# cnkuangshi/LightCTR

Hardware: AMD Instinct MI355X
Metric: examples/sec (whole node), FM training on synthetic Criteo-shaped sparse (higher is better)
Workload: dtype fp32; 1 GPU; model=FM k=16, ftrl fused update, global_batch=65536, num_features=16777216, num_fields=39, parallelism=single-gpu, hipGraph

## Files before the change

lightctr_amd/models/fm.py:

```python

from __future__ import annotations

from dataclasses import dataclass

import torch

from ..ops import fm_ref
from ..ops._extension import require_hip_ops, sort_ids, sort_ids_rec
from ..utils.checks import validate_csr_batch
from ..utils.metrics import auc_score


@dataclass
class FMHyper:
    num_features: int
    k: int = 16
    optimizer: str = "adagrad"
    lr: float = 0.1
    eps: float = 1e-8
    l2: float = 1e-5
    ftrl_alpha: float = 0.15
    ftrl_beta: float = 1.0
    ftrl_l1: float = 1e-4
    ftrl_l2: float = 1e-4
    ftrl_v: str = "adagrad"
    init_sigma: float = 0.01
    seed: int = 1234


class FMModel:

    def __init__(self, hyper: FMHyper, device: str = "cpu",
                 max_batch_nnz: int = 1 << 22):
        self.h = hyper
        self.device = torch.device(device)
        F, K = hyper.num_features, hyper.k
        assert K in (4, 8, 16, 32, 64), "K must divide the 64-lane wavefront"
        g = torch.Generator().manual_seed(hyper.seed)
        self.W = torch.zeros(F, device=self.device)
        self.V = (
            torch.randn(F, K, generator=g) * hyper.init_sigma
        ).to(self.device)
        self.gradW = torch.zeros_like(self.W)
        self.gradV = torch.zeros_like(self.V)
        self.nW = torch.zeros_like(self.W)
        self.nV = torch.zeros_like(self.V)
        if hyper.optimizer == "ftrl":
            self.zW = torch.zeros_like(self.W)
            self.zV = torch.zeros_like(self.V)
        nwords = (F + 63) // 64
        self.touched = torch.zeros(nwords, dtype=torch.int64, device=self.device)
        cap = min(F, max_batch_nnz)
        self.uniq = torch.zeros(cap, dtype=torch.int32, device=self.device)
        self.count = torch.zeros(1, dtype=torch.int32, device=self.device)
        self._use_hip = self.device.type == "cuda"
        self.backward_mode = "segment"
        self.segment_cap = 256
        self.fused_apply = False
        self.sort_impl = "onesweep"
        self.sort_status = torch.zeros(1, dtype=torch.int32,
                                       device=self.device)
        if self._use_hip:
            require_hip_ops()

    def forward(self, row_ptr, fids, vals):
        if self._use_hip:
            ops = require_hip_ops()
            pred, sumVX = ops.fm_forward(row_ptr, fids, vals, self.W, self.V)
        else:
            pred, sumVX = fm_ref.fm_forward_ref(row_ptr, fids, vals, self.W, self.V)
        return pred, sumVX

    def predict_proba(self, row_ptr, fids, vals):
        pred, _ = self.forward(row_ptr, fids, vals)
        return torch.sigmoid(torch.clamp(pred, -16, 16))

    def train_step(self, row_ptr, fids, vals, labels) -> torch.Tensor:
        B = row_ptr.numel() - 1
        scale = 1.0 / B
        validate_csr_batch(row_ptr, fids, vals, self.h.num_features)
        if self._use_hip:
            ops = require_hip_ops()
            if (self.backward_mode in ("segment", "segment_list")
                    and not self.fused_apply):
                tiled = (self.backward_mode == "segment"
                         and self._cap_tiles(ops))
                loss, dpred, sumVX, rec = ops.fm_forward_train(
                    row_ptr, fids, vals, self.W, self.V, labels, scale,
                    reset=self.count if tiled else None)
                self._segment_backward(ops, fids, sumVX, dpred, rec, tiled)
                return loss
            pred, sumVX = ops.fm_forward(row_ptr, fids, vals, self.W, self.V)
            loss, dpred = ops.logloss_grad(pred, labels, scale)
            if (self.backward_mode == "segment_emit"
                    and not self.fused_apply):
                self._segment_emit_backward(ops, row_ptr, fids, vals, sumVX,
                                            dpred)
                return loss
            if self.backward_mode in ("sorted", "segment", "segment_list",
                                      "segment_emit"):
                sorted_fids, perm = sort_ids(fids, self.h.num_features)
                gw, gv = ops.fm_backward_emit(row_ptr, fids, vals, self.V,
                                              sumVX, dpred)
                if self.fused_apply:
                    if (self.h.optimizer == "ftrl"
                            and self.h.ftrl_v == "adagrad"):
                        ops.fm_sorted_apply_fused(
                            sorted_fids, perm, gw, gv, self.gradW,
                            self.gradV, self.touched, self.W, self.V,
                            self.nW, self.nV, self.zW, None, 3,
                            self.h.ftrl_alpha, self.h.ftrl_beta,
                            self.h.ftrl_l1, self.h.ftrl_l2,
                            v_lr=self.h.lr, v_eps=self.h.eps,
                            v_l2=self.h.l2)
                    elif self.h.optimizer == "ftrl":
                        ops.fm_sorted_apply_fused(
                            sorted_fids, perm, gw, gv, self.gradW,
                            self.gradV, self.touched, self.W, self.V,
                            self.nW, self.nV, self.zW, self.zV, 2,
# ... 57 lines not shown
                                 self.h.lr, self.h.eps, self.h.l2)

    def _cap_tiles(self, ops) -> bool:
        tile, cap = ops.fm_segment_tile(), int(self.segment_cap)
        return cap <= tile and tile % cap == 0

    def _segment_pieces(self, ops, sorted_fids, worklist=True):
        nnz = sorted_fids.numel()
        cap = int(self.segment_cap)
        if worklist:
            lists = tuple(ops.segment_worklist(sorted_fids, cap, self.count))
        else:
            lists = (cap,)
        spill = self.uniq[: min(self.uniq.numel(), nnz // cap + 1)]
        mode = self._opt_mode()
        if mode == 1:
            knobs = (self.h.lr, self.h.eps, self.h.l2, 0.0)
        else:
            knobs = (self.h.ftrl_alpha, self.h.ftrl_beta, self.h.ftrl_l1,
                     self.h.ftrl_l2)
        tail = (*lists, self.gradW, self.gradV, spill,
                self.count, self.W, self.V, self.nW, self.nV,
                self.zW if mode != 1 else None,
                self.zV if mode == 2 else None, mode, *knobs)
        kw = dict(v_lr=self.h.lr, v_eps=self.h.eps, v_l2=self.h.l2)
        return spill, tail, kw

    def _segment_backward(self, ops, fids, sumVX, dpred, rec, tiled):
        if fids.numel() == 0:
            return
        sorted_fids, sorted_rec = sort_ids_rec(
            fids, rec, self.h.num_features, impl=self.sort_impl,
            status=self.sort_status)
        spill, tail, kw = self._segment_pieces(ops, sorted_fids,
                                               worklist=not tiled)
        reduce = (ops.fm_segment_tile_rec if tiled
                  else ops.fm_segment_apply_rec)
        reduce(sorted_fids, sorted_rec, sumVX, dpred, *tail, **kw)
        self._sparse_apply(ops, spill)

    def _segment_emit_backward(self, ops, row_ptr, fids, vals, sumVX, dpred):
        if fids.numel() == 0:
            return
        sorted_fids, perm = sort_ids(fids, self.h.num_features)
        gw, gv = ops.fm_backward_emit(row_ptr, fids, vals, self.V, sumVX,
                                      dpred)
        spill, tail, kw = self._segment_pieces(ops, sorted_fids)
        ops.fm_segment_apply(sorted_fids, perm, tail[0], tail[1], gw, gv,
                             *tail[2:], **kw)
        self._sparse_apply(ops, spill)

    def state_dict(self) -> dict:
        d = {"W": self.W, "V": self.V, "nW": self.nW, "nV": self.nV,
             "hyper": self.h.__dict__}
        if self.h.optimizer == "ftrl":
            d["zW"], d["zV"] = self.zW, self.zV
        return d

    def save(self, path: str) -> None:
        torch.save(self.state_dict(), path)

    def load(self, path: str) -> None:
        d = torch.load(path, map_location=self.device, weights_only=True)
        self.W.copy_(d["W"])
        self.V.copy_(d["V"])
        self.nW.copy_(d["nW"])
# ... 44 lines not shown
```

lightctr_amd/ops/_extension.py:

```python

from __future__ import annotations

import torch

_hip_ops = None
_import_error: Exception | None = None

try:
    from . import _hip_ops as _ext

    _hip_ops = _ext
except ImportError as e:
    _import_error = e


def has_hip_ops() -> bool:
    return _hip_ops is not None


def require_hip_ops():
    if _hip_ops is None:
        raise ImportError(
            "lightctr_amd HIP extension (_hip_ops) is not built but a GPU "
            "op was requested. Build it in-tree with "
            "`PYTORCH_ROCM_ARCH=gfx950 python setup.py build_ext --inplace`. "
            f"Original import error: {_import_error!r}"
        )
    return _hip_ops


class _LazyOps:

    def __getattr__(self, name):
        return getattr(require_hip_ops(), name)


hip_ops = _LazyOps()


def sort_ids(fids, upper: int):
    end_bit = max(1, int(upper - 1).bit_length())
    return require_hip_ops().radix_sort_index(fids, end_bit)


def sort_ids_rec(fids, rec, upper: int, impl: str = "onesweep", status=None):
    if impl not in ("onesweep", "rocprim"):
        raise ValueError(f"unknown sort impl {impl!r}")
    ops = require_hip_ops()
    end_bit = max(1, int(upper - 1).bit_length())
    if impl == "onesweep" and end_bit <= 31 and fids.numel() < (1 << 30):
        return ops.onesweep_sort_rec(fids, rec, end_bit, status)
    return ops.radix_sort_rec(fids, rec, end_bit)
```

lightctr_amd/ops/csrc/bindings.cpp:

```cpp
#include <torch/extension.h>
#include <ATen/cuda/CUDAContext.h>
#include <c10/cuda/CUDAException.h>

#include <cstdint>
#include <cstdio>
#include <cstdlib>
#include <cstring>
#include <limits>
#include <stdexcept>
#include <string>
#include <vector>

#include "launchers.h"

namespace {

#define CHK(x, ...) TORCH_CHECK(x, __VA_ARGS__)

void check_cuda_f32(const at::Tensor& t, const char* name) {
  CHK(t.is_cuda(), name, " must be on GPU");
  CHK(t.scalar_type() == at::kFloat, name, " must be fp32");
  CHK(t.is_contiguous(), name, " must be contiguous");
}

void check_cuda_i32(const at::Tensor& t, const char* name) {
  CHK(t.is_cuda(), name, " must be on GPU");
  CHK(t.scalar_type() == at::kInt, name, " must be int32");
  CHK(t.is_contiguous(), name, " must be contiguous");
}

void check_embed_k(int64_t K) {
  CHK(K == 4 || K == 8 || K == 16 || K == 32 || K == 64,
      "latent width K must be one of 4, 8, 16, 32, 64, got ", K);
}
// ... 1165 lines not shown
}

std::vector<at::Tensor> onesweep_sort_rec(at::Tensor keys, at::Tensor rec,
                                          int64_t end_bit,
                                          c10::optional<at::Tensor> status) {
  check_cuda_i32(keys, "keys");
  CHK(end_bit >= 1 && end_bit <= 31, "end_bit in [1,31]");
  CHK(keys.numel() < (1L << 30), "n must be below 2^30");
  const int n = (int)keys.numel();
  check_cuda_rec(rec, n, "rec");
  if (status.has_value()) {
    check_cuda_i32(*status, "status");
    CHK(status->numel() >= 1, "status must hold one word");
  }
  auto sorted = at::empty_like(keys);
  auto sorted_rec = at::empty_like(rec);
  if (n == 0) return {sorted, sorted_rec};
  auto st = status.has_value() ? *status : at::zeros({1}, keys.options());
  const unsigned long bytes =
      lightctr::onesweep_sort_work_bytes(n, (int)end_bit);
  auto work = at::empty({(long)bytes}, keys.options().dtype(at::kByte));
  at::Tensor keys_tmp, rec_tmp;
  if (end_bit > 8) {
    keys_tmp = at::empty_like(keys);
    rec_tmp = at::empty_like(rec);
  }
  lightctr::onesweep_sort_rec_launch(
      work.data_ptr(), keys.data_ptr<int>(), sorted.data_ptr<int>(),
      end_bit > 8 ? keys_tmp.data_ptr<int>() : nullptr, rec.data_ptr<int>(),
      sorted_rec.data_ptr<int>(),
      end_bit > 8 ? rec_tmp.data_ptr<int>() : nullptr, n, (int)end_bit,
      st.data_ptr<int>(), cur_stream());
  return {sorted, sorted_rec};
}


at::Tensor colsum(at::Tensor dZ) {
  check_cuda_f32(dZ, "dZ");
  const int M = (int)dZ.size(0), N = (int)dZ.size(1);
  auto db = at::empty({N}, dZ.options());
  lightctr::colsum_launch(dZ.data_ptr<float>(), db.data_ptr<float>(), M, N,
                          cur_stream());
  return db;
}

at::Tensor to_bf16(at::Tensor x) {
  check_cuda_f32(x, "x");
  auto y = at::empty_like(x, x.options().dtype(at::kBFloat16));
  lightctr::to_bf16_launch(x.data_ptr<float>(), y.data_ptr(), x.numel(),
                           cur_stream());
  return y;
}

void dense_adam(at::Tensor W, at::Tensor grad, at::Tensor m, at::Tensor v,
                c10::optional<at::Tensor> Wbf, c10::optional<at::Tensor> Wtbf,
                double lr, double beta1, double beta2, double eps,
                int64_t step, double l2) {
  check_cuda_f32(W, "W");
  const int rows = (int)W.size(0);
  const int cols = (int)(W.numel() / W.size(0));
  const float bc1 = 1.f - powf((float)beta1, (float)step);
  const float bc2 = 1.f - powf((float)beta2, (float)step);
  lightctr::dense_adam_launch(
      W.data_ptr<float>(), grad.data_ptr<float>(), m.data_ptr<float>(),
      v.data_ptr<float>(), Wbf.has_value() ? Wbf->data_ptr() : nullptr,
      Wtbf.has_value() ? Wtbf->data_ptr() : nullptr, rows, cols, (float)lr,
// ... 645 lines not shown
        py::arg("slab"), py::arg("acc"), py::arg("shadow"),
        py::arg("flags"), py::arg("updater"), py::arg("lr"),
        py::arg("lam"), py::arg("eps"));
  m.def("ps_dense_pack", &ps_dense_pack,
        "PS dense pull: slab -> fp32/fp16 payload (+ shadow = slab)",
        py::arg("slab"), py::arg("shadow"), py::arg("fp16"));
  m.def("sparse_ftrl_apply", &sparse_ftrl_apply,
        "generic sparse fused FTRL (runtime D; optional Adagrad on V)",
        py::arg("uniq"), py::arg("count"), py::arg("W"), py::arg("V"),
        py::arg("zW"), py::arg("nW"), py::arg("zV"), py::arg("nV"),
        py::arg("gradW"), py::arg("gradV"), py::arg("alpha"),
        py::arg("beta"), py::arg("l1"), py::arg("l2"),
        py::arg("v_adagrad") = 0, py::arg("v_lr") = 0.05,
        py::arg("v_eps") = 1e-8, py::arg("v_l2") = 1e-5,
        py::arg("Vh") = py::none());
  m.def("gemm_bf16", &gemm_bf16, "MFMA bf16 GEMM (C fp32), fused bias+act");
  m.def("gemm_bf16_full", &gemm_bf16_full,
        "MFMA bf16 GEMM returning (C fp32, C bf16)");
  m.def("act_backward", &act_backward, "dZ = dY*act'(Y), + bf16 mirror");
  m.def("inv_perm_i32", &inv_perm_i32, "inverse permutation (int32)");
  m.def("radix_sort_index", &radix_sort_index,
        "bit-range radix sort -> (sorted, perm)");
  m.def("radix_sort_rec", &radix_sort_rec,
        "bit-range radix sort with [n,2] int32 records as payload -> "
        "(sorted, sorted_rec)",
        py::arg("keys"), py::arg("rec"), py::arg("end_bit"));
  m.def("onesweep_sort_rec", &onesweep_sort_rec,
        "single-purpose onesweep sort with [n,2] int32 records as payload "
        "-> (sorted, sorted_rec); same result as radix_sort_rec",
        py::arg("keys"), py::arg("rec"), py::arg("end_bit"),
        py::arg("status") = py::none());
  m.def("onesweep_sort_tile", &lightctr::onesweep_sort_tile,
        "entries per tile of onesweep_sort_rec");
  m.def("colsum", &colsum, "bias gradient column sum");
  m.def("to_bf16", &to_bf16, "f32 -> bf16 convert");
  m.def("dense_adam", &dense_adam, "dense Adam + bf16 mirror refresh");
  m.def("dense_adagrad", &dense_adagrad,
        "dense Adagrad + bf16 mirror refresh");
  m.def("embed_gather", &embed_gather, "concat embedding gather -> bf16");
  m.def("embed_backward_emit", &embed_backward_emit,
        "per-entry embedding grads (gw, gv) for sorted apply");
  m.def("wide_forward", &wide_forward, "LR wide forward sum");
  m.def("w2v_negsample_step", &w2v_negsample_step,
        "fused CBOW negative-sampling train step (Hogwild)");
  m.def("quantile_encode", &quantile_encode, "int8 quantile encode");
  m.def("quantile_decode", &quantile_decode, "int8 quantile decode");
  m.def("lowbit_encode", &lowbit_encode, "1/2-bit sign quantize");
  m.def("lowbit_decode", &lowbit_decode, "1/2-bit dequantize");
  m.def("gbm_hist", &gbm_hist, "GBM per-node (grad,hess) histograms");
  m.def("gbm_forest", &gbm_forest,
        "compiled-forest inference: margin / leaf id / leaf feature id");
  m.def("gbm_forest_chunk_capacity", &lightctr::gbm_forest_chunk_capacity,
        "nodes per LDS chunk of the forest kernel");
  m.def("gbm_forest_max_register_classes",
        &lightctr::gbm_forest_max_register_classes,
        "largest class count with register accumulators");
  m.def("gbm_forest_rows_per_grid", &lightctr::gbm_forest_rows_per_grid,
        "rows one trip of the clamped grid covers");
  m.def("nfm_forward", &nfm_forward,
        "NFM bi-interaction fwd (wide, sumVX, vec, vec_bf16)");
  m.def("nfm_backward_emit", &nfm_backward_emit,
        "NFM per-entry grads for sorted apply");
  m.def("bitmap_compact", &bitmap_compact, "touched bitmap -> fid list");
  m.def("wg_probe", &wg_probe, "wgrad staging/tr-read debug probe");
  m.def("gemm_bf16_variant", &gemm_bf16_variant,
        "launch one named GEMM body directly; returns [C] or [C, Cbf]");
// ... 49 lines not shown
```

lightctr_amd/ops/csrc/fm_kernels.hip:

```cpp
#include <algorithm>
#include <cstdio>
#include "common.h"

namespace lightctr {

__device__ __forceinline__ void ftrl_step(float& w, float& z, float& n,
                                          float g, float alpha, float beta,
                                          float l1, float l2) {
  const float g2 = g * g;
  const float nold = n;
  const float sigma = (sqrtf(nold + g2) - sqrtf(nold)) / alpha;
  const float znew = z + g - sigma * w;
  const float nnew = nold + g2;
  z = znew;
  n = nnew;
  if (fabsf(znew) <= l1) {
    w = 0.f;
  } else {
    w = -(znew - copysignf(l1, znew)) / ((beta + sqrtf(nnew)) / alpha + l2);
  }
}

__device__ __forceinline__ void adagrad_step(float& w, float& n, float g_in,
                                             float lr, float eps, float l2) {
// ... 33 lines not shown
  float* zV;
  float p0, p1, p2, p3;
  float q0, q1, q2;
};

__device__ __forceinline__ void fm_opt_step_v(int opt_mode, float& v,
                                              float& n, float& z, float g,
                                              const FmOptArgs& oa) {
  if (opt_mode == 1) {
    adagrad_step(v, n, g, oa.p0, oa.p1, oa.p2);
  } else if (opt_mode == 3) {
    adagrad_step(v, n, g, oa.q0, oa.q1, oa.q2);
  } else {
    ftrl_step(v, z, n, g, oa.p0, oa.p1, oa.p2, oa.p3);
  }
}

__device__ __forceinline__ void fm_opt_step_w(int opt_mode, float& w,
                                              float& n, float& z, float g,
                                              const FmOptArgs& oa) {
  if (opt_mode == 1) {
    adagrad_step(w, n, g, oa.p0, oa.p1, oa.p2);
  } else {
    ftrl_step(w, z, n, g, oa.p0, oa.p1, oa.p2, oa.p3);
  }
}

__device__ __forceinline__ void logloss_grad_row(float z, float y, float scale,
                                                 float& loss, float& dpred) {
  loss = fmaxf(z, 0.f) - z * y + __logf(1.f + __expf(-fabsf(z)));
  dpred = (sigmoidf_clamped(z) - y) * scale;
}

template <int K, bool TRAIN>
__device__ __forceinline__ float fm_forward_row(
    const int* __restrict__ row_ptr, const int* __restrict__ fids,
    const float* __restrict__ vals, const float* __restrict__ W,
    const float* __restrict__ V, float* __restrict__ sumVX,
    int2* __restrict__ rec, int row, int lane) {
  constexpr int G = LCTR_WAVE / K;
  const int g = lane / K;
  const int k = lane % K;
  const int beg = row_ptr[row], end = row_ptr[row + 1];

  float sVX = 0.f;
  float sV2X2 = 0.f;
  float lin = 0.f;
  int j = beg + g;
  for (; j + 3 * G < end; j += 4 * G) {
    int f[4];
    float x[4], v[4], w[4];
#pragma unroll
    for (int u = 0; u < 4; ++u) {
      f[u] = fids[j + u * G];
      x[u] = vals[j + u * G];
    }
#pragma unroll
    for (int u = 0; u < 4; ++u) {
      v[u] = V[(size_t)f[u] * K + k];
      w[u] = (k == 0) ? W[f[u]] : 0.f;
    }
#pragma unroll
    for (int u = 0; u < 4; ++u) {
      if (TRAIN && k == 0)
        rec[j + u * G] = make_int2(row, __float_as_int(x[u]));
      const float vx = v[u] * x[u];
      sVX += vx;
      sV2X2 += vx * vx;
      lin += w[u] * x[u];
    }
  }
  for (; j < end; j += G) {
    const int fid = fids[j];
    const float x = vals[j];
    if (TRAIN && k == 0) rec[j] = make_int2(row, __float_as_int(x));
    const float vx = V[(size_t)fid * K + k] * x;
    sVX += vx;
    sV2X2 += vx * vx;
    if (k == 0) lin += W[fid] * x;
  }
  sVX = group_reduce_sum<K>(sVX);
  const float t = sVX * sVX;
  const float tot_t = wave_reduce_sum(t) * (1.f / G);
  const float tot_v2 = wave_reduce_sum(sV2X2);
  const float tot_lin = wave_reduce_sum(lin);
  if (lane < K) sumVX[(size_t)row * K + lane] = sVX;
  return tot_lin + 0.5f * (tot_t - tot_v2);
}

template <int K>
__global__ void fm_forward_kernel(const int* __restrict__ row_ptr,
                                  const int* __restrict__ fids,
                                  const float* __restrict__ vals,
                                  const float* __restrict__ W,
                                  const float* __restrict__ V,
                                  float* __restrict__ pred,
                                  float* __restrict__ sumVX, int B) {
  const int lane = threadIdx.x & (LCTR_WAVE - 1);
  const int row = blockIdx.x * (blockDim.x / LCTR_WAVE) + (threadIdx.x >> 6);
  if (row >= B) return;
  const float p = fm_forward_row<K, false>(row_ptr, fids, vals, W, V, sumVX,
                                           nullptr, row, lane);
  if (lane == 0) pred[row] = p;
}

template <int K>
__global__ void fm_forward_train_kernel(
    const int* __restrict__ row_ptr, const int* __restrict__ fids,
    const float* __restrict__ vals, const float* __restrict__ W,
    const float* __restrict__ V, const float* __restrict__ label, float scale,
    float* __restrict__ loss, float* __restrict__ dpred,
    float* __restrict__ sumVX, int2* __restrict__ rec, int B,
    int* __restrict__ reset) {
  const int lane = threadIdx.x & (LCTR_WAVE - 1);
  const int row = blockIdx.x * (blockDim.x / LCTR_WAVE) + (threadIdx.x >> 6);
  if (reset != nullptr && blockIdx.x == 0 && threadIdx.x == 0) *reset = 0;
  if (row >= B) return;
  const float p = fm_forward_row<K, true>(row_ptr, fids, vals, W, V, sumVX,
                                          rec, row, lane);
  if (lane == 0) {
    float l, d;
    logloss_grad_row(p, label[row], scale, l, d);
    loss[row] = l;
    dpred[row] = d;
  }
}

__global__ void logloss_grad_kernel(const float* __restrict__ pred,
                                    const float* __restrict__ label,
                                    float* __restrict__ loss,
                                    float* __restrict__ dpred, float scale,
                                    int B) {
  const int i = blockIdx.x * blockDim.x + threadIdx.x;
  if (i >= B) return;
  float l, d;
  logloss_grad_row(pred[i], label[i], scale, l, d);
  loss[i] = l;
  dpred[i] = d;
}

template <int K>
__global__ void fm_backward_kernel(
    const int* __restrict__ row_ptr, const int* __restrict__ fids,
    const float* __restrict__ vals, const float* __restrict__ V,
    const float* __restrict__ sumVX, const float* __restrict__ dpred,
    float* __restrict__ gradW, float* __restrict__ gradV,
    unsigned long long* __restrict__ touched, int B) {
  constexpr int G = LCTR_WAVE / K;
  const int lane = threadIdx.x & (LCTR_WAVE - 1);
  const int row = blockIdx.x * (blockDim.x / LCTR_WAVE) + (threadIdx.x >> 6);
  if (row >= B) return;
  const int g = lane / K;
  const int k = lane % K;
  const float d = dpred[row];
  const float sv = sumVX[(size_t)row * K + k];
  const int beg = row_ptr[row], end = row_ptr[row + 1];
  for (int j = beg + g; j < end; j += G) {
    const int fid = fids[j];
// ... 821 lines not shown
    ftrl_update(&V[off], &zV[off], &nV[off], gradV[off], alpha, beta, l1,
                l2);
  }
  gradV[off] = 0.f;
  if (k == 0) {
    ftrl_update(&W[fid], &zW[fid], &nW[fid], gradW[fid], alpha, beta, l1, l2);
    gradW[fid] = 0.f;
  }
}

static inline int waves_per_block() { return 4; }

void fm_forward_launch(const int* row_ptr, const int* fids, const float* vals,
                       const float* W, const float* V, float* pred,
                       float* sumVX, int B, int K, hipStream_t stream) {
  if (B <= 0) return;
  const int wpb = waves_per_block();
  dim3 block(wpb * LCTR_WAVE);
  dim3 grid((B + wpb - 1) / wpb);
  DISPATCH_K(K, hipLaunchKernelGGL((fm_forward_kernel<KC>), grid, block, 0,
                                   stream, row_ptr, fids, vals, W, V, pred,
                                   sumVX, B));
}

void fm_forward_train_launch(const int* row_ptr, const int* fids,
                             const float* vals, const float* W, const float* V,
                             const float* label, float scale, float* loss,
                             float* dpred, float* sumVX, int* rec, int B,
                             int K, int* reset, hipStream_t stream) {
  if (B <= 0) return;
  const int wpb = waves_per_block();
  dim3 block(wpb * LCTR_WAVE);
  dim3 grid((B + wpb - 1) / wpb);
  DISPATCH_K(K, hipLaunchKernelGGL((fm_forward_train_kernel<KC>), grid, block,
                                   0, stream, row_ptr, fids, vals, W, V, label,
                                   scale, loss, dpred, sumVX, (int2*)rec, B,
                                   reset));
}

void logloss_grad_launch(const float* pred, const float* label, float* loss,
                         float* dpred, float scale, int B,
                         hipStream_t stream) {
  if (B <= 0) return;
  dim3 block(256);
  dim3 grid((B + 255) / 256);
  hipLaunchKernelGGL(logloss_grad_kernel, grid, block, 0, stream, pred, label,
                     loss, dpred, scale, B);
}

void fm_backward_launch(const int* row_ptr, const int* fids, const float* vals,
                        const float* V, const float* sumVX, const float* dpred,
                        float* gradW, float* gradV, unsigned long long* touched,
                        int B, int K, hipStream_t stream) {
  if (B <= 0) return;
  const int wpb = waves_per_block();
  dim3 block(wpb * LCTR_WAVE);
  dim3 grid((B + wpb - 1) / wpb);
  DISPATCH_K(K, hipLaunchKernelGGL((fm_backward_kernel<KC>), grid, block, 0,
                                   stream, row_ptr, fids, vals, V, sumVX,
                                   dpred, gradW, gradV, touched, B));
}

void fm_backward_emit_launch(const int* row_ptr, const int* fids,
                             const float* vals, const float* V,
                             const float* sumVX, const float* dpred, float* gw,
                             float* gv, int B, int K, const int* pos,
                             hipStream_t stream) {
  if (B <= 0) return;
  const int wpb = waves_per_block();
  dim3 block(wpb * LCTR_WAVE);
// ... 256 lines not shown
```

lightctr_amd/ops/csrc/launchers.h:

```cpp
#pragma once

struct ihipStream_t;

namespace lightctr {

void fm_forward_launch(const int* row_ptr, const int* fids, const float* vals,
                       const float* W, const float* V, float* pred,
                       float* sumVX, int B, int K, ihipStream_t* stream);
void logloss_grad_launch(const float* pred, const float* label, float* loss,
                         float* dpred, float scale, int B,
                         ihipStream_t* stream);
void fm_backward_launch(const int* row_ptr, const int* fids, const float* vals,
                        const float* V, const float* sumVX, const float* dpred,
                        float* gradW, float* gradV, unsigned long long* touched,
                        int B, int K, ihipStream_t* stream);
void fm_backward_emit_launch(const int* row_ptr, const int* fids,
                             const float* vals, const float* V,
                             const float* sumVX, const float* dpred, float* gw,
                             float* gv, int B, int K, const int* pos,
                             ihipStream_t* stream);
void inv_perm_launch(const int* perm, int* inv, int n, ihipStream_t* stream);
void fm_sorted_apply_launch(const int* sorted_fids, const int* perm,
                            const float* gw, const float* gv, float* gradW,
                            float* gradV, unsigned long long* touched, int nnz,
                            int K, int opt_mode, float* V, float* W,
                            float* nW, float* zW, float* nV, float* zV,
                            float p0, float p1, float p2, float p3,
                            float q0, float q1, float q2,
                            int chunk, ihipStream_t* stream);
void fm_segment_apply_launch(const int* sorted_fids, const int* perm,
                             const int* piece_start, const int* n_pieces,
                             const float* gw, const float* gv, float* gradW,
                             float* gradV, int* spill, int* spill_count,
                             int spill_cap, int nnz, int K, int opt_mode,
                             float* V, float* W, float* nW, float* zW,
                             float* nV, float* zV, float p0, float p1,
                             float p2, float p3, float q0, float q1, float q2,
                             int num_cus, ihipStream_t* stream);
void fm_forward_train_launch(const int* row_ptr, const int* fids,
                             const float* vals, const float* W, const float* V,
                             const float* label, float scale, float* loss,
                             float* dpred, float* sumVX, int* rec, int B,
                             int K, int* reset, ihipStream_t* stream);
void fm_segment_recompute_launch(
    const int* sorted_fids, const int* rec, const float* sumVX,
    const float* dpred, int B, const int* piece_start, const int* n_pieces,
    float* gradW, float* gradV, int* spill, int* spill_count, int spill_cap,
    int nnz, int K, int opt_mode, float* V, float* W, float* nW, float* zW,
    float* nV, float* zV, float p0, float p1, float p2, float p3, float q0,
    float q1, float q2, int num_cus, ihipStream_t* stream);
int fm_segment_tile();
int fm_segment_split();
void fm_segment_tile_launch(const int* sorted_fids, const int* rec,
                            const float* sumVX, const float* dpred, int B,
                            int cap, float* gradW, float* gradV, int* spill,
                            int* spill_count, int spill_cap, int nnz, int K,
                            int opt_mode, float* V, float* W, float* nW,
                            float* zW, float* nV, float* zV, float p0,
                            float p1, float p2, float p3, float q0, float q1,
                            float q2, ihipStream_t* stream);
void bitmap_compact_launch(unsigned long long* bitmap, int nwords,
                           int* out_fids, int* out_count, int cap,
                           ihipStream_t* stream);

void ffm_forward_launch(const int* row_ptr, const int* fields, const int* fids,
                        const float* vals, const float* W, const float* V,
                        float* pred, int nfields, int B, int K,
                        ihipStream_t* stream);
void ffm_backward_launch(const int* row_ptr, const int* fields,
                         const int* fids, const float* vals, const float* V,
                         const float* dpred, float* gradW, float* gradV,
                         unsigned long long* touched, int nfields, int B,
                         int K, ihipStream_t* stream);

void ffm_sorted_backward_launch(const int* sorted_fids, const int* perm,
                                const int* row_of_entry, const int* row_ptr,
// ... 207 lines not shown
void lowbit_encode_launch(const float* x, unsigned int* words, float thresh,
                          int bits, long n, ihipStream_t* stream);
void lowbit_decode_launch(const unsigned int* words, float* x, float lo,
                          float hi, int bits, long n, ihipStream_t* stream);

void ps_dense_check_launch(const void* payload, int wire, const float* scale,
                           const float* table, int levels, long n,
                           int* flags, ihipStream_t* stream);
void ps_dense_apply_launch(const void* payload, int wire, const float* scale,
                           const float* table, int levels, float* slab,
                           float* acc, float* shadow, long n, int updater,
                           float lr, float lam, float eps, int* flags,
                           ihipStream_t* stream);
void ps_dense_pack_launch(const float* slab, void* out, int fp16,
                          float* shadow, long n, ihipStream_t* stream);

void iota_i32_launch(int* out, int n, ihipStream_t* stream);
unsigned long radix_sort_pairs_i32_temp_bytes(int n, int end_bit);
void radix_sort_pairs_i32_launch(void* temp, unsigned long temp_bytes,
                                 const int* keys_in, int* keys_out,
                                 const int* vals_in, int* vals_out, int n,
                                 int end_bit, ihipStream_t* stream);
unsigned long radix_sort_pairs_rec_temp_bytes(int n, int end_bit);
void radix_sort_pairs_rec_launch(void* temp, unsigned long temp_bytes,
                                 const int* keys_in, int* keys_out,
                                 const int* rec_in, int* rec_out, int n,
                                 int end_bit, ihipStream_t* stream);
int onesweep_sort_tile();
unsigned long onesweep_sort_work_bytes(int n, int end_bit);
void onesweep_sort_rec_launch(void* work, const int* keys_in, int* keys_out,
                              int* keys_tmp, const int* rec_in, int* rec_out,
                              int* rec_tmp, int n, int end_bit, int* status,
                              ihipStream_t* stream);
unsigned long segment_worklist_temp_bytes(int n);
void segment_worklist_launch(void* temp, unsigned long temp_bytes,
                             const int* sorted, int n, int cap,
                             int* piece_start, int* n_pieces, int* zero_me,
                             ihipStream_t* stream);

void gbm_hist_launch(const unsigned char* bins, const float* grad,
                     const float* hess, const int* node_of_row, float* hist,
                     int N, int D, int n_nodes, ihipStream_t* stream);
int gbm_forest_chunk_capacity();
int gbm_forest_max_register_classes();
long gbm_forest_rows_per_grid();
void gbm_forest_launch(const float* X, const void* nodes, const int* tree_off,
                       const int* tree_class, const int* leaf_base,
                       const void* chunks, int n_chunks, void* out, long N,
                       int D, int T, int K, int max_depth, int fid_offset,
                       int mode, ihipStream_t* stream);

int knn_max_k();
int knn_max_sub();
int knn_max_dim();
long knn_slice_rows(long n, long nq);
long pq_adc_lds_bytes(int n_sub, int ncb);
void pq_lut_launch(const float* Q, const float* C, float* lut, long nq,
                   int n_sub, int ncb, int d_sub, int ip,
                   ihipStream_t* stream);
void pq_adc_topk_launch(const float* lut, const unsigned char* codes,
                        long stride, long N, long nq, int n_sub, int ncb,
                        int k, long slice_rows, int n_slices, void* partial,
                        int* ids, float* dist, ihipStream_t* stream);
void flat_topk_launch(const float* X, long stride, long N, int dim,
                      const float* Q, long nq, const int* cand, long n_items,
                      int ip, int k, long slice_rows, int n_slices,
// ... 15 lines not shown
```

lightctr_amd/ops/csrc/sort_kernels.hip:

```cpp
#include <algorithm>

#include <rocprim/device/device_radix_sort.hpp>
#include <rocprim/device/device_select.hpp>
#include <rocprim/iterator/counting_iterator.hpp>
#include <rocprim/iterator/transform_iterator.hpp>

#include "common.h"

namespace lightctr {

__global__ void iota_i32_kernel(int* __restrict__ out, int n) {
  int i = blockIdx.x * blockDim.x + threadIdx.x;
  if (i < n) out[i] = i;
}

void iota_i32_launch(int* out, int n, hipStream_t stream) {
  if (n <= 0) return;
  int threads = 256;
  int blocks = (n + threads - 1) / threads;
  hipLaunchKernelGGL(iota_i32_kernel, dim3(blocks), dim3(threads), 0, stream,
                     out, n);
}

size_t radix_sort_pairs_i32_temp_bytes(int n, int end_bit) {
// ... 9 lines not shown
                                 const int* keys_in, int* keys_out,
                                 const int* vals_in, int* vals_out, int n,
                                 int end_bit, hipStream_t stream) {
  LCTR_CHECK_HIP(rocprim::radix_sort_pairs(temp, temp_bytes, keys_in,
                                           keys_out, vals_in, vals_out,
                                           (size_t)n, 0u, (unsigned)end_bit,
                                           stream, false));
}

using SortRec = unsigned long long;

size_t radix_sort_pairs_rec_temp_bytes(int n, int end_bit) {
  size_t bytes = 0;
  (void)rocprim::radix_sort_pairs(nullptr, bytes, (const int*)nullptr,
                                  (int*)nullptr, (const SortRec*)nullptr,
                                  (SortRec*)nullptr, (size_t)n, 0u,
                                  (unsigned)end_bit, (hipStream_t)0, false);
  return bytes;
}

void radix_sort_pairs_rec_launch(void* temp, size_t temp_bytes,
                                 const int* keys_in, int* keys_out,
                                 const int* rec_in, int* rec_out, int n,
                                 int end_bit, hipStream_t stream) {
  LCTR_CHECK_HIP(rocprim::radix_sort_pairs(
      temp, temp_bytes, keys_in, keys_out, (const SortRec*)rec_in,
      (SortRec*)rec_out, (size_t)n, 0u, (unsigned)end_bit, stream, false));
}

constexpr int kOsRadix = 256;
constexpr int kOsMaxPasses = 4;
constexpr int kOsCtrlWords = kOsMaxPasses * kOsRadix + kOsMaxPasses;
static_assert(kOsCtrlWords * 4 % 16 == 0, "memset block is 16-byte padded");
constexpr unsigned kOsCountMask = 0x3fffffffu;
constexpr unsigned kOsAggregate = 1u << 30;
constexpr unsigned kOsPrefix = 2u << 30;
constexpr unsigned kOsSpinLimit = 1u << 20;
constexpr int kOsHistMaxThreads = 1024;
constexpr int kOsHistMaxBlocks = 256;
constexpr int kOsThreads = 512;
constexpr int kOsItems = 8;
constexpr int kOsWindow = 4;

#define OS_RLX_AGENT __ATOMIC_RELAXED, __HIP_MEMORY_SCOPE_AGENT

__global__ __launch_bounds__(kOsHistMaxThreads) void onesweep_hist_kernel(
    const int* __restrict__ keys, int n, int passes, unsigned keymask,
    unsigned* ghist, uint4* state, long state_vec4) {
  __shared__ unsigned h[kOsMaxPasses * kOsRadix];
  const int tid = threadIdx.x, threads = blockDim.x;
  for (int i = tid; i < passes * kOsRadix; i += threads) h[i] = 0;
  const long gstride = (long)gridDim.x * threads;
  for (long i = (long)blockIdx.x * threads + tid; i < state_vec4; i += gstride)
    state[i] = make_uint4(0u, 0u, 0u, 0u);
  __syncthreads();
  const int stride = (int)gstride;
#pragma unroll 4
  for (int i = blockIdx.x * threads + tid; i < n; i += stride) {
    const unsigned k = (unsigned)keys[i] & keymask;
#pragma unroll
    for (int p = 0; p < kOsMaxPasses; ++p)
      if (p < passes) atomicAdd(&h[p * kOsRadix + ((k >> (8 * p)) & 255u)], 1u);
  }
  __syncthreads();
  for (int i = tid; i < passes * kOsRadix; i += threads) {
    const unsigned c = h[i];
    if (c) atomicAdd(&ghist[i], c);
  }
}

__device__ __forceinline__ unsigned os_scan256(unsigned v, unsigned* wsum,
                                               int tid) {
  const int lane = tid & 63, w = tid >> 6;
  unsigned incl = v;
#pragma unroll
  for (int o = 1; o < 64; o <<= 1) {
    const unsigned t = __shfl_up(incl, o);
    if (lane >= o) incl += t;
  }
  if (tid < kOsRadix && lane == 63) wsum[w] = incl;
  __syncthreads();
  unsigned add = 0;
  if (tid < kOsRadix)
    for (int k = 0; k < w; ++k) add += wsum[k];
  return incl - v + add;
}

template <int THREADS, int IPT>
constexpr int os_smem_bytes() {
  constexpr int rank_bytes = (THREADS / 64) * kOsRadix * 12 + kOsRadix * 4;
  constexpr int tile_bytes = THREADS * IPT * 12;
  return (tile_bytes > rank_bytes ? tile_bytes : rank_bytes) + kOsRadix * 4 +
         48;
}

// ... 168 lines not shown
  }
}

template <int THREADS, int IPT>
void os_scatter_launch(int tiles, const int* keys_in, const SortRec* rec_in,
                       int* keys_out, SortRec* rec_out, int n, int shift,
                       unsigned keymask, const unsigned* ghist,
                       unsigned* ticket, unsigned* state, int* status,
                       hipStream_t stream) {
  constexpr int smem = os_smem_bytes<THREADS, IPT>();
  static_assert(smem <= 160 * 1024, "tile does not fit the LDS");
  auto kernel = onesweep_scatter_kernel<THREADS, IPT>;
  if (smem > 64 * 1024) {
    static const hipError_t raised = hipFuncSetAttribute(
        (const void*)kernel, hipFuncAttributeMaxDynamicSharedMemorySize, smem);
    LCTR_CHECK_HIP(raised);
  }
  hipLaunchKernelGGL(kernel, dim3(tiles), dim3(THREADS), smem, stream, keys_in,
                     rec_in, keys_out, rec_out, n, shift, keymask, ghist,
                     ticket, state, status);
}

int onesweep_sort_tile() { return kOsThreads * kOsItems; }

static int os_passes(int end_bit) { return (end_bit + 7) / 8; }

size_t onesweep_sort_work_bytes(int n, int end_bit) {
  const size_t tile = kOsThreads * kOsItems;
  const size_t tiles = ((size_t)n + tile - 1) / tile;
  return (size_t)kOsCtrlWords * 4 +
         (size_t)os_passes(end_bit) * tiles * kOsRadix * 4;
}

void onesweep_sort_rec_launch(void* work, const int* keys_in, int* keys_out,
                              int* keys_tmp, const int* rec_in, int* rec_out,
                              int* rec_tmp, int n, int end_bit, int* status,
                              hipStream_t stream) {
  if (n <= 0) return;
  const int passes = os_passes(end_bit);
  const int tile = kOsThreads * kOsItems;
  const int tiles = (n + tile - 1) / tile;
  const unsigned keymask = (1u << end_bit) - 1u;
  unsigned* ghist = (unsigned*)work;
  unsigned* tickets = ghist + kOsMaxPasses * kOsRadix;
  unsigned* state = ghist + kOsCtrlWords;
  const size_t pass_words = (size_t)tiles * kOsRadix;
  LCTR_CHECK_HIP(hipMemsetAsync(work, 0, (size_t)kOsCtrlWords * 4, stream));
  const int hist_blocks = std::min(
      kOsHistMaxBlocks,
      (n + kOsHistMaxThreads * 8 - 1) / (kOsHistMaxThreads * 8));
  hipLaunchKernelGGL(onesweep_hist_kernel, dim3(hist_blocks),
                     dim3(kOsHistMaxThreads), 0, stream, keys_in, n, passes,
                     keymask, ghist, (uint4*)state,
                     (long)(passes * pass_words / 4));
  const int* ksrc = keys_in;
  const SortRec* rsrc = (const SortRec*)rec_in;
  for (int p = 0; p < passes; ++p) {
    const bool to_out = ((passes - 1 - p) & 1) == 0;
    int* kdst = to_out ? keys_out : keys_tmp;
    SortRec* rdst = (SortRec*)(to_out ? rec_out : rec_tmp);
    os_scatter_launch<kOsThreads, kOsItems>(
        tiles, ksrc, rsrc, kdst, rdst, n, 8 * p, keymask,
        ghist + p * kOsRadix, tickets + p, state + p * pass_words, status,
        stream);
    ksrc = kdst;
    rsrc = rdst;
  }
}

struct PieceStartFlag {
  const int* sorted;
  int cap_mask;
  int* zero_me;
  __device__ bool operator()(int e) const {
    if (e == 0) {
      if (zero_me) *zero_me = 0;
      return true;
    }
    return (e & cap_mask) == 0 || sorted[e] != sorted[e - 1];
  }
};

using PieceFlagIter =
    rocprim::transform_iterator<rocprim::counting_iterator<int>,
                                PieceStartFlag, bool>;

size_t segment_worklist_temp_bytes(int n) {
  size_t bytes = 0;
  const rocprim::counting_iterator<int> idx(0);
  (void)rocprim::select(nullptr, bytes, idx,
                        PieceFlagIter(idx, PieceStartFlag{nullptr, 0, nullptr}),
                        (int*)nullptr, (int*)nullptr, (size_t)n,
                        (hipStream_t)0, false);
  return bytes;
}

void segment_worklist_launch(void* temp, size_t temp_bytes, const int* sorted,
                             int n, int cap, int* piece_start, int* n_pieces,
                             int* zero_me, hipStream_t stream) {
  const rocprim::counting_iterator<int> idx(0);
// ... 8 lines not shown
```

Before: 205.3 million examples/sec.

## Overlap record sort with FM forward on a side stream, building records in histogram

Adds a fused path where the onesweep sort of (fid, record) runs on a side stream in parallel with the FM training forward. The histogram kernel now reads the CSR directly and writes the records itself, so the forward no longer emits them and the sort no longer waits for the forward. A single-block zero kernel replaces the memset of the sort control block. This trades extra stream/event fork-join overhead (inside a hipGraph) and contention between concurrent kernels for hiding the sort latency behind forward compute.

```diff
diff --git a/lightctr_amd/models/fm.py b/lightctr_amd/models/fm.py
--- a/lightctr_amd/models/fm.py
+++ b/lightctr_amd/models/fm.py
@@ -6,7 +6,8 @@
 import torch
 
 from ..ops import fm_ref
-from ..ops._extension import require_hip_ops, sort_ids, sort_ids_rec
+from ..ops._extension import (require_hip_ops, sort_end_bit, sort_ids,
+                              sort_ids_rec)
 from ..utils.checks import validate_csr_batch
 from ..utils.metrics import auc_score
 
@@ -60,6 +61,7 @@
         self.sort_impl = "onesweep"
         self.sort_status = torch.zeros(1, dtype=torch.int32,
                                        device=self.device)
+        self.overlap_sort = True
         if self._use_hip:
             require_hip_ops()
 
@@ -85,6 +87,19 @@
                     and not self.fused_apply):
                 tiled = (self.backward_mode == "segment"
                          and self._cap_tiles(ops))
+                end_bit = sort_end_bit(self.h.num_features)
+                if (self.overlap_sort and self.sort_impl == "onesweep"
+                        and end_bit <= 31 and fids.numel() < (1 << 30)):
+                    loss, dpred, sumVX, sorted_fids, sorted_rec = (
+                        ops.fm_forward_train_sorted(
+                            row_ptr, fids, vals, self.W, self.V, labels,
+                            scale, end_bit,
+                            reset=self.count if tiled else None,
+                            status=self.sort_status,
+                            overlap=self.overlap_sort != "serial"))
+                    self._segment_reduce(ops, sorted_fids, sorted_rec, sumVX,
+                                         dpred, tiled)
+                    return loss
                 loss, dpred, sumVX, rec = ops.fm_forward_train(
                     row_ptr, fids, vals, self.W, self.V, labels, scale,
                     reset=self.count if tiled else None)
@@ -208,6 +223,13 @@
         sorted_fids, sorted_rec = sort_ids_rec(
             fids, rec, self.h.num_features, impl=self.sort_impl,
             status=self.sort_status)
+        self._segment_reduce(ops, sorted_fids, sorted_rec, sumVX, dpred,
+                             tiled)
+
+    def _segment_reduce(self, ops, sorted_fids, sorted_rec, sumVX, dpred,
+                        tiled):
+        if sorted_fids.numel() == 0:
+            return
         spill, tail, kw = self._segment_pieces(ops, sorted_fids,
                                                worklist=not tiled)
         reduce = (ops.fm_segment_tile_rec if tiled
diff --git a/lightctr_amd/ops/_extension.py b/lightctr_amd/ops/_extension.py
--- a/lightctr_amd/ops/_extension.py
+++ b/lightctr_amd/ops/_extension.py
@@ -38,8 +38,12 @@
 hip_ops = _LazyOps()
 
 
+def sort_end_bit(upper: int) -> int:
+    return max(1, int(upper - 1).bit_length())
+
+
 def sort_ids(fids, upper: int):
-    end_bit = max(1, int(upper - 1).bit_length())
+    end_bit = sort_end_bit(upper)
     return require_hip_ops().radix_sort_index(fids, end_bit)
 
 
@@ -47,7 +51,7 @@
     if impl not in ("onesweep", "rocprim"):
         raise ValueError(f"unknown sort impl {impl!r}")
     ops = require_hip_ops()
-    end_bit = max(1, int(upper - 1).bit_length())
+    end_bit = sort_end_bit(upper)
     if impl == "onesweep" and end_bit <= 31 and fids.numel() < (1 << 30):
         return ops.onesweep_sort_rec(fids, rec, end_bit, status)
     return ops.radix_sort_rec(fids, rec, end_bit)
diff --git a/lightctr_amd/ops/csrc/bindings.cpp b/lightctr_amd/ops/csrc/bindings.cpp
--- a/lightctr_amd/ops/csrc/bindings.cpp
+++ b/lightctr_amd/ops/csrc/bindings.cpp
@@ -1,5 +1,6 @@
 #include <torch/extension.h>
 #include <ATen/cuda/CUDAContext.h>
+#include <ATen/cuda/CUDAEvent.h>
 #include <c10/cuda/CUDAException.h>
 
 #include <cstdint>
@@ -1231,6 +1232,129 @@
       end_bit > 8 ? rec_tmp.data_ptr<int>() : nullptr, n, (int)end_bit,
       st.data_ptr<int>(), cur_stream());
   return {sorted, sorted_rec};
+}
+
+at::Tensor fm_records(at::Tensor row_ptr, at::Tensor vals) {
+  check_cuda_i32(row_ptr, "row_ptr");
+  check_cuda_f32(vals, "vals");
+  CHK(row_ptr.numel() >= 1, "row_ptr must hold B + 1 offsets");
+  const int B = (int)row_ptr.numel() - 1;
+  auto rec = at::empty({vals.numel(), 2}, row_ptr.options());
+  if (vals.numel() == 0) return rec;
+  lightctr::fm_records_launch(row_ptr.data_ptr<int>(), vals.data_ptr<float>(),
+                              rec.data_ptr<int>(), B, cur_stream());
+  return rec;
+}
+
+struct CsrSortBuffers {
+  at::Tensor sorted, sorted_rec, work, keys_tmp, rec_tmp, status;
+};
+
+void check_csr_sort(const at::Tensor& row_ptr, const at::Tensor& fids,
+                    const at::Tensor& vals, int64_t end_bit,
+                    const c10::optional<at::Tensor>& status) {
+  check_cuda_i32(row_ptr, "row_ptr");
+  check_cuda_i32(fids, "fids");
+  check_cuda_f32(vals, "vals");
+  CHK(row_ptr.numel() >= 1, "row_ptr must hold B + 1 offsets");
+  CHK(vals.numel() == fids.numel(), "vals must have one value per entry");
+  CHK(end_bit >= 1 && end_bit <= 31, "end_bit in [1,31]");
+  CHK(fids.numel() < (1L << 30), "n must be below 2^30");
+  if (status.has_value()) {
+    check_cuda_i32(*status, "status");
+    CHK(status->numel() >= 1, "status must hold one word");
+  }
+}
+
+CsrSortBuffers alloc_csr_sort(const at::Tensor& fids, int64_t end_bit,
+                              const c10::optional<at::Tensor>& status) {
+  CsrSortBuffers b;
+  const long n = fids.numel();
+  b.sorted = at::empty_like(fids);
+  b.sorted_rec = at::empty({n, 2}, fids.options());
+  if (n == 0) return b;
+  b.status = status.has_value() ? *status : at::zeros({1}, fids.options());
+  const unsigned long bytes =
+      lightctr::onesweep_sort_work_bytes((int)n, (int)end_bit);
+  b.work = at::empty({(long)bytes}, fids.options().dtype(at::kByte));
+  b.rec_tmp = at::empty({n, 2}, fids.options());
+  if (end_bit > 8) b.keys_tmp = at::empty_like(fids);
+  return b;
+}
+
+void launch_csr_sort(const CsrSortBuffers& b, const at::Tensor& row_ptr,
+                     const at::Tensor& fids, const at::Tensor& vals,
+                     int64_t end_bit, ihipStream_t* stream) {
+  lightctr::onesweep_sort_csr_launch(
+      b.work.data_ptr(), row_ptr.data_ptr<int>(), fids.data_ptr<int>(),
+      vals.data_ptr<float>(), (int)row_ptr.numel() - 1,
+      b.sorted.data_ptr<int>(),
+      end_bit > 8 ? b.keys_tmp.data_ptr<int>() : nullptr,
+      b.sorted_rec.data_ptr<int>(), b.rec_tmp.data_ptr<int>(),
+      (int)fids.numel(), (int)end_bit, b.status.data_ptr<int>(), stream);
+}
+
+std::vector<at::Tensor> onesweep_sort_csr(at::Tensor row_ptr, at::Tensor fids,
+                                          at::Tensor vals, int64_t end_bit,
+                                          c10::optional<at::Tensor> status) {
+  check_csr_sort(row_ptr, fids, vals, end_bit, status);
+  auto b = alloc_csr_sort(fids, end_bit, status);
+  if (fids.numel() > 0 && row_ptr.numel() > 1)
+    launch_csr_sort(b, row_ptr, fids, vals, end_bit, cur_stream());
+  return {b.sorted, b.sorted_rec};
+}
+
+std::vector<at::Tensor> fm_forward_train_sorted(
+    at::Tensor row_ptr, at::Tensor fids, at::Tensor vals, at::Tensor W,
+    at::Tensor V, at::Tensor label, double scale, int64_t end_bit,
+    c10::optional<at::Tensor> reset, c10::optional<at::Tensor> status,
+    bool overlap) {
+  check_csr_sort(row_ptr, fids, vals, end_bit, status);
+  check_cuda_f32(W, "W");
+  check_cuda_f32(V, "V");
+  check_cuda_f32(label, "label");
+  const int B = (int)row_ptr.numel() - 1;
+  const int K = (int)V.size(1);
+  const long nnz = fids.numel();
+  CHK(label.numel() == B, "label must have one value per row");
+  int* reset_ptr = nullptr;
+  if (reset.has_value()) {
+    check_cuda_i32(*reset, "reset");
+    CHK(reset->numel() >= 1, "reset must hold one int");
+    reset_ptr = reset->data_ptr<int>();
+    if (B <= 0) reset->zero_();
+  }
+  auto loss = at::empty({B}, W.options());
+  auto dpred = at::empty({B}, W.options());
+  auto sumVX = at::empty({B, K}, W.options());
+  auto b = alloc_csr_sort(fids, end_bit, status);
+  if (B <= 0) return {loss, dpred, sumVX, b.sorted, b.sorted_rec};
+  const auto forward = [&](ihipStream_t* stream) {
+    lightctr::fm_forward_train_launch(
+        row_ptr.data_ptr<int>(), fids.data_ptr<int>(), vals.data_ptr<float>(),
+        W.data_ptr<float>(), V.data_ptr<float>(), label.data_ptr<float>(),
+        (float)scale, loss.data_ptr<float>(), dpred.data_ptr<float>(),
+        sumVX.data_ptr<float>(), nullptr, B, K, reset_ptr, stream);
+  };
+  if (nnz == 0) {
+    forward(cur_stream());
+  } else if (!overlap) {
+    forward(cur_stream());
+    launch_csr_sort(b, row_ptr, fids, vals, end_bit, cur_stream());
+  } else {
+    const auto main = at::cuda::getCurrentCUDAStream();
+    const auto side =
+        at::cuda::getStreamFromPool(false, main.device_index());
+    at::cuda::CUDAEvent fork, join;
+    fork.record(main);
+    fork.block(side);
+    launch_csr_sort(b, row_ptr, fids, vals, end_bit,
+                    (ihipStream_t*)side.stream());
+    forward((ihipStream_t*)main.stream());
+    join.record(side);
+    join.block(main);
+  }
+  return {loss, dpred, sumVX, b.sorted, b.sorted_rec};
 }
 
 
@@ -1942,6 +2066,21 @@
         py::arg("status") = py::none());
   m.def("onesweep_sort_tile", &lightctr::onesweep_sort_tile,
         "entries per tile of onesweep_sort_rec");
+  m.def("fm_records", &fm_records,
+        "records of a CSR batch: rec[j] = (row of j, bits of vals[j])",
+        py::arg("row_ptr"), py::arg("vals"));
+  m.def("onesweep_sort_csr", &onesweep_sort_csr,
+        "onesweep sort of a CSR batch's (fid, record) stream, the records "
+        "made by the histogram kernel -> (sorted, sorted_rec)",
+        py::arg("row_ptr"), py::arg("fids"), py::arg("vals"),
+        py::arg("end_bit"), py::arg("status") = py::none());
+  m.def("fm_forward_train_sorted", &fm_forward_train_sorted,
+        "FM training forward and the record sort of the batch, side by side "
+        "with overlap -> (loss, dpred, sumVX, sorted_fids, sorted_rec)",
+        py::arg("row_ptr"), py::arg("fids"), py::arg("vals"), py::arg("W"),
+        py::arg("V"), py::arg("label"), py::arg("scale"), py::arg("end_bit"),
+        py::arg("reset") = py::none(), py::arg("status") = py::none(),
+        py::arg("overlap") = true);
   m.def("colsum", &colsum, "bias gradient column sum");
   m.def("to_bf16", &to_bf16, "f32 -> bf16 convert");
   m.def("dense_adam", &dense_adam, "dense Adam + bf16 mirror refresh");
diff --git a/lightctr_amd/ops/csrc/fm_kernels.hip b/lightctr_amd/ops/csrc/fm_kernels.hip
--- a/lightctr_amd/ops/csrc/fm_kernels.hip
+++ b/lightctr_amd/ops/csrc/fm_kernels.hip
@@ -89,7 +89,7 @@
   dpred = (sigmoidf_clamped(z) - y) * scale;
 }
 
-template <int K, bool TRAIN>
+template <int K, bool REC>
 __device__ __forceinline__ float fm_forward_row(
     const int* __restrict__ row_ptr, const int* __restrict__ fids,
     const float* __restrict__ vals, const float* __restrict__ W,
@@ -119,22 +119,22 @@
     }
 #pragma unroll
     for (int u = 0; u < 4; ++u) {
-      if (TRAIN && k == 0)
+      if (REC && k == 0)
         rec[j + u * G] = make_int2(row, __float_as_int(x[u]));
       const float vx = v[u] * x[u];
       sVX += vx;
       sV2X2 += vx * vx;
-      lin += w[u] * x[u];
+      lin = fmaf(w[u], x[u], lin);
     }
   }
   for (; j < end; j += G) {
     const int fid = fids[j];
     const float x = vals[j];
-    if (TRAIN && k == 0) rec[j] = make_int2(row, __float_as_int(x));
+    if (REC && k == 0) rec[j] = make_int2(row, __float_as_int(x));
     const float vx = V[(size_t)fid * K + k] * x;
     sVX += vx;
     sV2X2 += vx * vx;
-    if (k == 0) lin += W[fid] * x;
+    if (k == 0) lin = fmaf(W[fid], x, lin);
   }
   sVX = group_reduce_sum<K>(sVX);
   const float t = sVX * sVX;
@@ -161,7 +161,7 @@
   if (lane == 0) pred[row] = p;
 }
 
-template <int K>
+template <int K, bool REC>
 __global__ void fm_forward_train_kernel(
     const int* __restrict__ row_ptr, const int* __restrict__ fids,
     const float* __restrict__ vals, const float* __restrict__ W,
@@ -173,14 +173,25 @@
   const int row = blockIdx.x * (blockDim.x / LCTR_WAVE) + (threadIdx.x >> 6);
   if (reset != nullptr && blockIdx.x == 0 && threadIdx.x == 0) *reset = 0;
   if (row >= B) return;
-  const float p = fm_forward_row<K, true>(row_ptr, fids, vals, W, V, sumVX,
-                                          rec, row, lane);
+  const float p = fm_forward_row<K, REC>(row_ptr, fids, vals, W, V, sumVX,
+                                         rec, row, lane);
   if (lane == 0) {
     float l, d;
     logloss_grad_row(p, label[row], scale, l, d);
     loss[row] = l;
     dpred[row] = d;
   }
+}
+
+__global__ void fm_records_kernel(const int* __restrict__ row_ptr,
+                                  const float* __restrict__ vals,
+                                  int2* __restrict__ rec, int B) {
+  const int lane = threadIdx.x & (LCTR_WAVE - 1);
+  const int row = blockIdx.x * (blockDim.x / LCTR_WAVE) + (threadIdx.x >> 6);
+  if (row >= B) return;
+  const int end = row_ptr[row + 1];
+  for (int j = row_ptr[row] + lane; j < end; j += LCTR_WAVE)
+    rec[j] = make_int2(row, __float_as_int(vals[j]));
 }
 
 __global__ void logloss_grad_kernel(const float* __restrict__ pred,
@@ -1068,10 +1079,27 @@
   const int wpb = waves_per_block();
   dim3 block(wpb * LCTR_WAVE);
   dim3 grid((B + wpb - 1) / wpb);
-  DISPATCH_K(K, hipLaunchKernelGGL((fm_forward_train_kernel<KC>), grid, block,
-                                   0, stream, row_ptr, fids, vals, W, V, label,
-                                   scale, loss, dpred, sumVX, (int2*)rec, B,
-                                   reset));
+  if (rec != nullptr) {
+    DISPATCH_K(K, hipLaunchKernelGGL((fm_forward_train_kernel<KC, true>), grid,
+                                     block, 0, stream, row_ptr, fids, vals, W,
+                                     V, label, scale, loss, dpred, sumVX,
+                                     (int2*)rec, B, reset));
+  } else {
+    DISPATCH_K(K, hipLaunchKernelGGL((fm_forward_train_kernel<KC, false>),
+                                     grid, block, 0, stream, row_ptr, fids,
+                                     vals, W, V, label, scale, loss, dpred,
+                                     sumVX, (int2*)nullptr, B, reset));
+  }
+}
+
+void fm_records_launch(const int* row_ptr, const float* vals, int* rec, int B,
+                       hipStream_t stream) {
+  if (B <= 0) return;
+  const int wpb = waves_per_block();
+  dim3 block(wpb * LCTR_WAVE);
+  dim3 grid((B + wpb - 1) / wpb);
+  hipLaunchKernelGGL(fm_records_kernel, grid, block, 0, stream, row_ptr, vals,
+                     (int2*)rec, B);
 }
 
 void logloss_grad_launch(const float* pred, const float* label, float* loss,
diff --git a/lightctr_amd/ops/csrc/launchers.h b/lightctr_amd/ops/csrc/launchers.h
--- a/lightctr_amd/ops/csrc/launchers.h
+++ b/lightctr_amd/ops/csrc/launchers.h
@@ -42,6 +42,8 @@
                              const float* label, float scale, float* loss,
                              float* dpred, float* sumVX, int* rec, int B,
                              int K, int* reset, ihipStream_t* stream);
+void fm_records_launch(const int* row_ptr, const float* vals, int* rec, int B,
+                       ihipStream_t* stream);
 void fm_segment_recompute_launch(
     const int* sorted_fids, const int* rec, const float* sumVX,
     const float* dpred, int B, const int* piece_start, const int* n_pieces,
@@ -315,6 +317,11 @@
                               int* keys_tmp, const int* rec_in, int* rec_out,
                               int* rec_tmp, int n, int end_bit, int* status,
                               ihipStream_t* stream);
+void onesweep_sort_csr_launch(void* work, const int* row_ptr,
+                              const int* keys_in, const float* vals, int B,
+                              int* keys_out, int* keys_tmp, int* rec_out,
+                              int* rec_tmp, int n, int end_bit, int* status,
+                              ihipStream_t* stream);
 unsigned long segment_worklist_temp_bytes(int n);
 void segment_worklist_launch(void* temp, unsigned long temp_bytes,
                              const int* sorted, int n, int cap,
diff --git a/lightctr_amd/ops/csrc/sort_kernels.hip b/lightctr_amd/ops/csrc/sort_kernels.hip
--- a/lightctr_amd/ops/csrc/sort_kernels.hip
+++ b/lightctr_amd/ops/csrc/sort_kernels.hip
@@ -65,12 +65,14 @@
 constexpr int kOsMaxPasses = 4;
 constexpr int kOsCtrlWords = kOsMaxPasses * kOsRadix + kOsMaxPasses;
 static_assert(kOsCtrlWords * 4 % 16 == 0, "memset block is 16-byte padded");
+static_assert(kOsCtrlWords / 4 <= 1024, "one block zeroes the control block");
 constexpr unsigned kOsCountMask = 0x3fffffffu;
 constexpr unsigned kOsAggregate = 1u << 30;
 constexpr unsigned kOsPrefix = 2u << 30;
 constexpr unsigned kOsSpinLimit = 1u << 20;
 constexpr int kOsHistMaxThreads = 1024;
 constexpr int kOsHistMaxBlocks = 256;
+constexpr int kOsHistRecMaxBlocks = 512;
 constexpr int kOsThreads = 512;
 constexpr int kOsItems = 8;
 constexpr int kOsWindow = 4;
@@ -94,6 +96,65 @@
 #pragma unroll
     for (int p = 0; p < kOsMaxPasses; ++p)
       if (p < passes) atomicAdd(&h[p * kOsRadix + ((k >> (8 * p)) & 255u)], 1u);
+  }
+  __syncthreads();
+  for (int i = tid; i < passes * kOsRadix; i += threads) {
+    const unsigned c = h[i];
+    if (c) atomicAdd(&ghist[i], c);
+  }
+}
+
+constexpr int kOsHistRows = 4;
+
+__global__ __launch_bounds__(kOsHistMaxThreads) void onesweep_hist_rec_kernel(
+    const int* __restrict__ row_ptr, const int* __restrict__ keys,
+    const float* __restrict__ vals, int2* __restrict__ rec, int B, int n,
+    int passes, unsigned keymask, unsigned* ghist, uint4* state, long state_vec4) {
+  __shared__ unsigned h[kOsMaxPasses * kOsRadix];
+  const int tid = threadIdx.x, threads = blockDim.x;
+  for (int i = tid; i < passes * kOsRadix; i += threads) h[i] = 0;
+  const long gstride = (long)gridDim.x * threads;
+  for (long i = (long)blockIdx.x * threads + tid; i < state_vec4; i += gstride)
+    state[i] = make_uint4(0u, 0u, 0u, 0u);
+  __syncthreads();
+  const int lane = tid & 63;
+  const int wstride = (int)(gstride >> 6);
+  auto count = [&](unsigned k) {
+    k &= keymask;
+#pragma unroll
+    for (int p = 0; p < kOsMaxPasses; ++p)
+      if (p < passes) atomicAdd(&h[p * kOsRadix + ((k >> (8 * p)) & 255u)], 1u);
+  };
+  for (long row0 = ((long)blockIdx.x * threads + tid) >> 6; row0 < B;
+       row0 += (long)kOsHistRows * wstride) {
+    int row[kOsHistRows], j[kOsHistRows], end[kOsHistRows], k[kOsHistRows],
+        x[kOsHistRows];
+#pragma unroll
+    for (int u = 0; u < kOsHistRows; ++u) {
+      const long r = row0 + (long)u * wstride;
+      const bool live = r < B;
+      row[u] = (int)r;
+      j[u] = live ? max(row_ptr[r], 0) + lane : 0;
+      end[u] = live ? min(row_ptr[r + 1], n) : 0;
+    }
+#pragma unroll
+    for (int u = 0; u < kOsHistRows; ++u) {
+      if (j[u] < end[u]) {
+        k[u] = keys[j[u]];
+        x[u] = __float_as_int(vals[j[u]]);
+      }
+    }
+#pragma unroll
+    for (int u = 0; u < kOsHistRows; ++u) {
+      if (j[u] < end[u]) {
+        rec[j[u]] = make_int2(row[u], x[u]);
+        count((unsigned)k[u]);
+      }
+      for (int jj = j[u] + 64; jj < end[u]; jj += 64) {
+        rec[jj] = make_int2(row[u], __float_as_int(vals[jj]));
+        count((unsigned)keys[jj]);
+      }
+    }
   }
   __syncthreads();
   for (int i = tid; i < passes * kOsRadix; i += threads) {
@@ -328,6 +389,30 @@
          (size_t)os_passes(end_bit) * tiles * kOsRadix * 4;
 }
 
+static void os_scatter_passes(unsigned* ghist, const int* keys_in,
+                              int* keys_out, int* keys_tmp,
+                              const SortRec* rec_in, SortRec* rec_out,
+                              SortRec* rec_tmp, int n, int passes, int tiles,
+                              unsigned keymask, int* status,
+                              hipStream_t stream) {
+  unsigned* tickets = ghist + kOsMaxPasses * kOsRadix;
+  unsigned* state = ghist + kOsCtrlWords;
+  const size_t pass_words = (size_t)tiles * kOsRadix;
+  const int* ksrc = keys_in;
+  const SortRec* rsrc = rec_in;
+  for (int p = 0; p < passes; ++p) {
+    const bool to_out = ((passes - 1 - p) & 1) == 0;
+    int* kdst = to_out ? keys_out : keys_tmp;
+    SortRec* rdst = to_out ? rec_out : rec_tmp;
+    os_scatter_launch<kOsThreads, kOsItems>(
+        tiles, ksrc, rsrc, kdst, rdst, n, 8 * p, keymask,
+        ghist + p * kOsRadix, tickets + p, state + p * pass_words, status,
+        stream);
+    ksrc = kdst;
+    rsrc = rdst;
+  }
+}
+
 void onesweep_sort_rec_launch(void* work, const int* keys_in, int* keys_out,
                               int* keys_tmp, const int* rec_in, int* rec_out,
                               int* rec_tmp, int n, int end_bit, int* status,
@@ -338,30 +423,50 @@
   const int tiles = (n + tile - 1) / tile;
   const unsigned keymask = (1u << end_bit) - 1u;
   unsigned* ghist = (unsigned*)work;
-  unsigned* tickets = ghist + kOsMaxPasses * kOsRadix;
-  unsigned* state = ghist + kOsCtrlWords;
-  const size_t pass_words = (size_t)tiles * kOsRadix;
   LCTR_CHECK_HIP(hipMemsetAsync(work, 0, (size_t)kOsCtrlWords * 4, stream));
   const int hist_blocks = std::min(
       kOsHistMaxBlocks,
       (n + kOsHistMaxThreads * 8 - 1) / (kOsHistMaxThreads * 8));
   hipLaunchKernelGGL(onesweep_hist_kernel, dim3(hist_blocks),
                      dim3(kOsHistMaxThreads), 0, stream, keys_in, n, passes,
-                     keymask, ghist, (uint4*)state,
-                     (long)(passes * pass_words / 4));
-  const int* ksrc = keys_in;
-  const SortRec* rsrc = (const SortRec*)rec_in;
-  for (int p = 0; p < passes; ++p) {
-    const bool to_out = ((passes - 1 - p) & 1) == 0;
-    int* kdst = to_out ? keys_out : keys_tmp;
-    SortRec* rdst = (SortRec*)(to_out ? rec_out : rec_tmp);
-    os_scatter_launch<kOsThreads, kOsItems>(
-        tiles, ksrc, rsrc, kdst, rdst, n, 8 * p, keymask,
-        ghist + p * kOsRadix, tickets + p, state + p * pass_words, status,
-        stream);
-    ksrc = kdst;
-    rsrc = rdst;
-  }
+                     keymask, ghist, (uint4*)(ghist + kOsCtrlWords),
+                     (long)(passes * (size_t)tiles * kOsRadix / 4));
+  os_scatter_passes(ghist, keys_in, keys_out, keys_tmp, (const SortRec*)rec_in,
+                    (SortRec*)rec_out, (SortRec*)rec_tmp, n, passes, tiles,
+                    keymask, status, stream);
+}
+
+__global__ __launch_bounds__(kOsCtrlWords / 4) void onesweep_zero_kernel(
+    uint4* ctrl) {
+  ctrl[threadIdx.x] = make_uint4(0u, 0u, 0u, 0u);
+}
+
+void onesweep_sort_csr_launch(void* work, const int* row_ptr,
+                              const int* keys_in, const float* vals, int B,
+                              int* keys_out, int* keys_tmp, int* rec_out,
+                              int* rec_tmp, int n, int end_bit, int* status,
+                              hipStream_t stream) {
+  if (n <= 0 || B <= 0) return;
+  const int passes = os_passes(end_bit);
+  const int tile = kOsThreads * kOsItems;
+  const int tiles = (n + tile - 1) / tile;
+  const unsigned keymask = (1u << end_bit) - 1u;
+  unsigned* ghist = (unsigned*)work;
+  hipLaunchKernelGGL(onesweep_zero_kernel, dim3(1), dim3(kOsCtrlWords / 4), 0,
+                     stream, (uint4*)work);
+  const int wpb = kOsHistMaxThreads / 64;
+  const int hist_blocks = std::min(
+      kOsHistRecMaxBlocks, (B + wpb * kOsHistRows - 1) / (wpb * kOsHistRows));
+  int* rec_csr = (passes & 1) ? rec_tmp : rec_out;
+  hipLaunchKernelGGL(onesweep_hist_rec_kernel, dim3(hist_blocks),
+                     dim3(kOsHistMaxThreads), 0, stream, row_ptr, keys_in, vals,
+                     (int2*)rec_csr, B, n, passes, keymask, ghist,
+                     (uint4*)(ghist + kOsCtrlWords),
+                     (long)(passes * (size_t)tiles * kOsRadix / 4));
+  os_scatter_passes(ghist, keys_in, keys_out, keys_tmp,
+                    (const SortRec*)rec_csr, (SortRec*)rec_out,
+                    (SortRec*)rec_tmp, n, passes, tiles, keymask, status,
+                    stream);
 }
 
 struct PieceStartFlag {
```

New measurement: 212.1 million examples/sec, median of 6. 3.3% higher.
